# zivy/LSQRRecipes

Measured on AMD Instinct MI355X. Metric: RANSAC hypotheses/sec + final-fit residual, 10M pts, 1/2/4/8 GPU, higher is better.
Workload: dtype f64; 1 GPU; PlaneParametersEstimator + RANSAC, 10000000 points, 50% outliers, delta=0.50 (BASELINE.json configs[1]); points=10000000, streams=4, world_size=1, collectives=none (single GPU), repeats=3

## Files before the change

include/lsqr_hip.h:

```cpp
#ifndef LSQR_HIP_H
#define LSQR_HIP_H

#include <stddef.h>
#include <stdint.h>

#ifdef __cplusplus
extern "C" {
#endif

#if defined(__GNUC__)
#define LSQR_API __attribute__((visibility("default")))
#else
#define LSQR_API
#endif

typedef enum {
  LSQR_OK = 0,
  LSQR_EMPTY = 1,
  LSQR_ERR_INVALID = 2,
  LSQR_ERR_NO_DEVICE = 3,
  LSQR_ERR_HIP = 4,
  LSQR_ERR_STATE = 5
} lsqr_status;

// ... 281 lines not shown
                               uint8_t *consensus_out, lsqr_ransac_info *info);

LSQR_API int lsqr_ransac_exhaustive(lsqr_ctx *ctx, double *params_out, uint8_t *consensus_out,
                                    lsqr_ransac_info *info);
LSQR_API int lsqr_replay_init(size_t n, int k, double p, uint64_t state[6]);
LSQR_API size_t lsqr_replay(size_t n, int k, double p, const uint32_t *subsets,
                            const uint8_t *valid, const uint32_t *votes, size_t H,
                            uint64_t base_index, void *dedup_set, uint64_t state[6]);
LSQR_API void *lsqr_dedup_create(int k);
LSQR_API void lsqr_dedup_destroy(void *set);

LSQR_API int lsqr_set_option(lsqr_ctx *ctx, const char *name, int value);

LSQR_API int lsqr_index_info(const lsqr_ctx *ctx, uint64_t out[4]);

LSQR_API int lsqr_scan_workload(lsqr_ctx *ctx, uint32_t *bound_out, uint64_t out[8]);

LSQR_API int lsqr_scan_work(lsqr_ctx *ctx, uint64_t out[8]);

LSQR_API int lsqr_scan_pairs_counted(lsqr_ctx *ctx, uint64_t out[4]);

LSQR_API int lsqr_lm_persist_info(const lsqr_ctx *ctx, uint64_t out[8], uint64_t *trace, uint32_t trace_cap,
                                  uint32_t *trace_n);

LSQR_API int lsqr_profile_enable(lsqr_ctx *ctx, int on);
LSQR_API int lsqr_profile_get(lsqr_ctx *ctx, int kernel_id, uint64_t *launches, double *total_ms);
LSQR_API int lsqr_profile_reset(lsqr_ctx *ctx);

#ifdef __cplusplus
}
// ... 3 lines not shown
```

lsqrrecipes_amd/_lib.py:

```python
import ctypes as C
import os

import numpy as np

_HERE = os.path.dirname(os.path.abspath(__file__))
LIB_PATH = os.path.join(_HERE, "liblsqr_hip.so")

OK, EMPTY, ERR_INVALID, ERR_NO_DEVICE, ERR_HIP, ERR_STATE = range(6)
PLANE, SPHERE, LINE, DENSE, US_SINGLE, US_POINTER, ABSOR, PIVOT, RAY, LINE2D, PHANTOM = 1, 2, 3, 4, 5, 6, 7, 8, 9, 10, 11
LS_ALGEBRAIC, LS_GEOMETRIC = 0, 1
LS_ANALYTIC, LS_ITERATIVE = 0, 1
KERNEL_IDS = {"sample": 0, "estimate": 1, "scan": 2, "mask": 3, "moments": 4, "solve": 5,
              "index": 6, "absmax": 7}


def assign_dense_chunk(n):
    return 256 if n <= 32 else 128


class LsqrError(RuntimeError):
    def __init__(self, status, msg):
        RuntimeError.__init__(self, "lsqr_hip status %d: %s" % (status, msg))
        self.status = status

# ... 140 lines not shown
    "lsqr_multi_last_error": (C.c_char_p, [C.c_void_p]),
    "lsqr_multi_set_model": (C.c_int, [C.c_void_p, C.POINTER(ModelCfg)]),
    "lsqr_multi_upload": (C.c_int, [C.c_void_p, C.c_void_p, C.c_size_t, C.c_size_t]),
    "lsqr_multi_batch_fit": (C.c_int, [C.c_void_p, C.c_uint64, C.c_uint64, C.c_size_t, C.c_void_p, C.c_void_p,
                                       C.POINTER(RansacInfo)]),
    "lsqr_multi_ransac": (C.c_int, [C.c_void_p, C.c_double, C.c_uint64, C.c_void_p, C.c_void_p,
                                    C.POINTER(RansacInfo)]),
    "lsqr_ransac_exhaustive": (C.c_int, [_ctx, C.c_void_p, C.c_void_p, C.POINTER(RansacInfo)]),
    "lsqr_replay_init": (C.c_int, [C.c_size_t, C.c_int, C.c_double, _u64p]),
    "lsqr_replay": (C.c_size_t, [C.c_size_t, C.c_int, C.c_double, C.c_void_p, C.c_void_p,
                                 C.c_void_p, C.c_size_t, C.c_uint64, C.c_void_p, _u64p]),
    "lsqr_dedup_create": (C.c_void_p, [C.c_int]),
    "lsqr_dedup_destroy": (None, [C.c_void_p]),
    "lsqr_set_option": (C.c_int, [_ctx, C.c_char_p, C.c_int]),
    "lsqr_index_info": (C.c_int, [_ctx, _u64p]),
    "lsqr_scan_workload": (C.c_int, [_ctx, C.c_void_p, _u64p]),
    "lsqr_scan_work": (C.c_int, [_ctx, _u64p]),
    "lsqr_scan_pairs_counted": (C.c_int, [_ctx, _u64p]),
    "lsqr_lm_persist_info": (C.c_int, [_ctx, _u64p, _u64p, C.c_uint32, C.POINTER(C.c_uint32)]),
    "lsqr_profile_enable": (C.c_int, [_ctx, C.c_int]),
    "lsqr_profile_get": (C.c_int, [_ctx, C.c_int, _u64p, _dp]),
    "lsqr_profile_reset": (C.c_int, [_ctx]),
}

_lib = None


def load():
    global _lib
    if _lib is None:
# ... 21 lines not shown
```

lsqrrecipes_amd/context.py:

```python
import ctypes as C

import numpy as np

from . import _lib as L


class Context:
    def __init__(self, device=0):
        self._lib = L.load()
        h = C.c_void_p()
        st = self._lib.lsqr_ctx_create(int(device), C.byref(h))
        if st != L.OK:
            raise L.LsqrError(st, "lsqr_ctx_create(device=%d): %s" % (
                device, self._lib.lsqr_status_string(st).decode()))
        self._h = h
        self.device = device
        self.cfg = None
        self._keep = None

    def close(self):
        if getattr(self, "_h", None):
            self._lib.lsqr_ctx_destroy(self._h)
            self._h = None

# ... 702 lines not shown
        self._chk(self._lib.lsqr_profile_enable(self._h, int(on)))
        self._chk(self._lib.lsqr_profile_reset(self._h))

    def profile_get(self, name):
        n = C.c_uint64(0)
        ms = C.c_double(0)
        self._chk(self._lib.lsqr_profile_get(self._h, L.KERNEL_IDS[name], C.byref(n), C.byref(ms)))
        return n.value, ms.value

    def index_info(self):
        out = (C.c_uint64 * 4)()
        self._chk(self._lib.lsqr_index_info(self._h, out))
        return {"built": bool(out[0]), "observations": int(out[1]), "cells": int(out[2]),
                "cell_points": int(out[3])}

    def scan_workload(self, want_bounds=False):
        H = self._lib.lsqr_num_hypotheses(self._h)
        ub = np.zeros(H, dtype=np.uint32) if want_bounds else None
        out = (C.c_uint64 * 8)()
        self._chk(self._lib.lsqr_scan_workload(self._h, L.ptr(ub), out))
        r = {"pairs": int(out[0]), "level1_evaluations": int(out[1]), "cells": int(out[2]),
             "cell_points": int(out[3]), "bounded": bool(out[4]), "pilots": int(out[5]),
             "second_pass": int(out[6]), "pairs_counted": int(out[7])}
        if want_bounds:
            r["bounds"] = ub
        return r

    def scan_work(self):
        out = (C.c_uint64 * 8)()
        self._chk(self._lib.lsqr_scan_work(self._h, out))
# ... 123 lines not shown
```

lsqrrecipes_amd/csrc/cells.h:

```cpp
#pragma once
#include <hip/hip_runtime.h>
#include <stdint.h>

#include "models.h"

#pragma clang diagnostic ignored "-Winline-asm"

namespace lsqr {

constexpr int kCellPtsMin = 128;
constexpr uint32_t kGroupPad = 4, kCellPad = 16;
constexpr uint32_t kBlockPad = 6;
constexpr uint32_t kQueues = 32;
constexpr uint32_t kQueuePitch = 1088;

struct CellBox {
  float c[3];
  float h[3];
  float pad[2];
};
struct CellSlab {
  float e[3];
  float iee;
  float tmid, tspan;
// ... 1036 lines not shown
      const float a0 = d < D ? (float)(p0[d < D ? d : 0] - off) : 0.0f;
      const float a1 = d < D ? (float)(p1[d < D ? d : 0] - off) : 0.0f;
      xs[p][d].x = (d < D && !(i0 < ns)) ? __builtin_nanf("") : a0;
      xs[p][d].y = (d < D && !(i1 < ns)) ? __builtin_nanf("") : a1;
    }
    v2f q = {0.0f, 0.0f};
    if constexpr (requires { CM::XQ; }) {
      q = xs[p][D - 1] * xs[p][D - 1];
#pragma unroll
      for (int d = D - 2; d >= 0; d--) q = __builtin_elementwise_fma(xs[p][d], xs[p][d], q);
    }
    xs[p][3] = q;
  }
}

template <class CM, int PP, int CPT, int BS, bool LDSB = false>
__global__ __launch_bounds__(BS) __attribute__((amdgpu_waves_per_eu(CPT == 1 ? (PP >= 8 ? 4 : CM::MIN_WAVES) : 1, 8))) void k_scan_cells(const double *__restrict__ sorted, size_t ns,
                                                    const CellBox *__restrict__ boxes,
                                                    uint32_t ncells, const double *__restrict__ sp,
                                                    const float *__restrict__ rows,
                                                    const float *__restrict__ spf, uint32_t H,
                                                    ModelConsts mc, CellConsts cc,
                                                    uint32_t *__restrict__ votes,
                                                    uint32_t *__restrict__ next_tile, uint32_t grab,
                                                    uint32_t hsplit, const uint32_t *__restrict__ h_dev) {
  typedef typename CM::M M;
  constexpr int NB = CM::NB;
  if (h_dev) {
    const uint32_t hd = *h_dev;
    H = hd < H ? hd : H;
  }
  constexpr int SPD = M::SP;
  constexpr int ROW = CM::ROW, NR4 = ROW / 4;
  constexpr int NR2 = CM::ROW2 / 4;
  static_assert(ROW % 4 == 0, "hypothesis rows are fetched as 16-byte loads");
  extern __shared__ uint32_t s_cnt[];
  for (uint32_t h = threadIdx.x; h < H; h += BS) s_cnt[h] = 0;
  __syncthreads();
  const int lane = threadIdx.x & 63;
  float *s_bc = (float *)(s_cnt + ((H + 3) & ~3u)) + (size_t)(threadIdx.x >> 6) * 512;
// ... 27 lines not shown
    const uint32_t hbeg = (un - wt * hsplit) * hseg, hend = hbeg + hseg < H ? hbeg + hseg : H;
    if (hbeg >= H) continue;
    v2f xs[CPT][PP][4];
    CellBox bx[CPT];
    double ctr[CPT][3];
#pragma unroll
    for (int q = 0; q < CPT; q++) {
      const uint32_t cell = wt * CPT + q;
      if (cell < ncells) {
        bx[q] = boxes[cell];
      } else {
        for (int d = 0; d < 3; d++) bx[q].c[d] = 0.0f, bx[q].h[d] = __builtin_nanf("");
      }
#pragma unroll
      for (int d = 0; d < 3; d++) ctr[q][d] = (double)bx[q].c[d];
      cells_load<CM, PP>(sorted, ns, (size_t)cell, lane, ctr[q], xs[q]);
    }
    float4 nxt[NR4];
    {
      const uint32_t hl = hbeg + lane;
      const float4 *r4 = (const float4 *)(rows + (size_t)(hl < H ? hl : 0) * ROW);
#pragma unroll
      for (int k = 0; k < NR4; k++) nxt[k] = r4[k];
    }
    float4 nxt2[NR2 ? NR2 : 1];
    if constexpr (NR2 > 0) {
      const uint32_t hl = hbeg + lane;
      const float4 *r4 = (const float4 *)(spf + (size_t)(hl < H ? hl : 0) * M::SPF + CM::ROW2_OFF);
#pragma unroll
      for (int k = 0; k < NR2; k++) nxt2[k] = r4[k];
    }
// ... 622 lines not shown
    float bc[NB];
    (void)CM::level1(hy, bx, ctr, w.cc, bc);
    base += 64;
    const bool more = base < jhi;
    if (more) hy = hyp_gather<CM>(w.hyps, block_ids(base, s_id + (par ^ 64)));
    cells_filter_squares(bc);
    uint32_t accv = 0;
    cells_survivors<CM, PP, slots_dup(LDSB), Ids::List, EXACT>(
        xs, bc, w.s_bc, surv, lane, w.sorted, w.ns, (size_t)cell, w.sp, w.mc, accv, s_id + par, w.s_amb);
    if (accv) atomicAdd(&w.s_cnt[s_id[par + lane]], accv);
    if (!more) break;
    par ^= 64;
  }
}

template <class CM, int PP, int BS, bool LDSB, PairsForm F>
__global__ __launch_bounds__(BS) __attribute__((amdgpu_waves_per_eu(PP >= 8 ? 4 : CM::MIN_WAVES, 8))) void k_scan_pairs(
    const double *__restrict__ sorted, size_t ns, const CellBox *__restrict__ boxes, uint32_t ncells,
    const double *__restrict__ sp, const float *__restrict__ rows, const float *__restrict__ spf, uint32_t H,
    ModelConsts mc, CellConsts cc, uint32_t *__restrict__ vpart, uint32_t vstride,
    const uint32_t *__restrict__ h_dev, const uint8_t *__restrict__ cnt, uint32_t gstride, const uint32_t *__restrict__ cost,
    const uint32_t *__restrict__ csum, uint32_t nchunks, uint32_t h_off, const float4 *__restrict__ hyps,
    unsigned long long *__restrict__ ambc) {
  static_assert(pairs_form_exists<CM, LDSB, F>());
  constexpr bool PREP = prepared(F), LEAN = lean(F), PACK = packed(F);
  typedef typename CM::M M;
  constexpr int NB = CM::NB;
  constexpr int SPD = M::SP;
  [[maybe_unused]] constexpr int ROW = CM::ROW;
  constexpr int NR2 = CM::ROW2 / 4;
  constexpr int NR4 = [] {
    if constexpr (PREP) return (int)HypWords<CM>::N4;
    else return (int)CM::ROW / 4;
  }();
  if (h_dev) {
    const uint32_t hd = *h_dev > h_off ? *h_dev - h_off : 0u;
    H = hd < H ? hd : H;
  }
  extern __shared__ uint32_t s_cnt[];
// ... 135 lines not shown
    const CellBox bx = boxes[cell];
    double ctr[3];
#pragma unroll
    for (int d = 0; d < 3; d++) ctr[d] = (double)bx.c[d];
    if constexpr (LEAN && PP >= 4) {
#pragma unroll
      for (int d = 0; d < 3; d++) {
        const unsigned long long u = __builtin_bit_cast(unsigned long long, ctr[d]);
        uint32_t l, m;
        asm("s_nop 0\n\tv_readfirstlane_b32 %0, %1\n\ts_nop 1" : "=s"(l) : "v"((uint32_t)u));
        asm("s_nop 0\n\tv_readfirstlane_b32 %0, %1\n\ts_nop 1" : "=s"(m) : "v"((uint32_t)(u >> 32)));
        ctr[d] = __builtin_bit_cast(double, (unsigned long long)m << 32 | l);
      }
    }
    v2f xs[PP][4];
    cells_load<CM, PP>(sorted, ns, (size_t)cell, lane, ctr, xs);
    if constexpr (PACK) {
      pairs_cell_packed<CM, PP, LDSB, recheck(F) ? Exact::Band : Exact::Cell>(w, cell, bx, ctr, xs, jlo, jhi);
      cell++;
      continue;
    }
    if constexpr (LEAN) {
      typename CM::Hyp hy;
      {
        float4 r[NR4], r2[1];
        load_rows((uint32_t)__builtin_ctzll(gm), r, r2);
        hy = hyp_from<CM>(r);
      }
      while (gm && budget) {
        const int g = __builtin_ctzll(gm);
        gm &= gm - 1;
// ... 167 lines not shown
```

lsqrrecipes_amd/csrc/lsqr_hip.hip:

```cpp
#include <hip/hip_runtime.h>

#include <algorithm>
#include <atomic>
#include <chrono>
#include <cmath>
#include <cstdarg>
#include <cstddef>
#include <cstdio>
#include <cstdlib>
#include <cstring>
#include <limits>
#include <set>
#include <thread>
#include <string>
#include <type_traits>
#include <utility>
#include <vector>

#include "../../include/lsqr_hip.h"
#include "devbuf.h"
#include "options.h"
#include "kernels.h"
#include "models_nd.h"
#include "dense.h"
// ... 151 lines not shown

  DevBuf<double> d_sorted;
  DevBuf<uint32_t> d_queues;
  DevBuf<CellBox> d_boxes;
  uint32_t super_merge = 0;
  size_t n_sorted = 0;
  uint32_t n_cells = 0, cell_pts = 0;
  bool index_valid = false;
  bool index_failed = false;
  DevBuf<char> d_idx_scratch;
  int kd_build_levels = 0, index_kd_levels = 0;
  DevBuf<CellAxis> d_axis;
  DevBuf<float> d_cellT;
  bool axis_valid = false;
  DevBuf<CellSlab> d_slab;

  DevBuf<uint32_t> d_ub;
  struct {
    bool valid = false, packed = false, slab = false;
    uint32_t H = 0, h_off = 0, gstride = 0;
    const uint32_t *h_dev = nullptr;
  } last_count;
  DevBuf<uint8_t> d_paircnt;
  DevBuf<uint32_t> d_paircost;
  DevBuf<uint32_t> d_vpart;
  DevBuf<float4> d_hyps;
  DevBuf<unsigned long long> d_pairmask;
  DevBuf<unsigned long long> d_ambcnt;
  bool amb_reset = false;
  bool amb_counted = false;
// ... 438 lines not shown
    if (c->lanes[i]) {
      (void)hipStreamSynchronize(c->lanes[i]->stream);
      for (BatchSlotState &s : c->lanes[i]->slots) s.busy = false;
    }
}

void drop_index(lsqr_ctx *c) {
  c->h16_valid = false;
  c->us16_valid = false;
  c->h16_nomem = c->us16_nomem = false;
  c->n_sorted = 0;
  c->n_cells = 0;
  c->index_valid = false;
  c->index_kd_levels = 0;
  c->axis_valid = false;
  c->last_count.valid = false;
}

template <int D>
int run_bounds(lsqr_ctx *c) {
  if (c->bounds_valid) return LSQR_OK;
  const int nb = grid_for(c->n, 256 * 16, 1024);
  BoundsRow *rows = (BoundsRow *)c->d_partials.get();
  static_assert(sizeof(BoundsRow) == 64, "BoundsRow is 8 words");
  {
    ProfScope ps(c, KID_ABSMAX);
    hipLaunchKernelGGL((k_bounds<D>), dim3(nb), dim3(256), 0, c->stream, c->d_data, c->stride, c->n, rows);
  }
  HIPCHK(c, hipGetLastError());
  hipLaunchKernelGGL(k_bounds_final, dim3(1), dim3(256), 0, c->stream, rows, nb, rows + 1024);
// ... 148 lines not shown
        double xabs;
        memcpy(&xabs, &hb.amax, sizeof xabs);
        hipLaunchKernelGGL(k_cell_slabs, dim3((c->n_cells + 255) / 256), dim3(256), 0, c->stream, c->d_boxes, c->d_axis,
                           c->d_cellT, c->n_sorted, c->n_cells, cell_pts, xabs, (uint32_t)c->opt.slab_gate, c->d_slab);
      }
      IDXCHK(hipGetLastError());
      c->axis_valid = true;
    }
  }
#undef IDXCHK
  c->index_kd_levels = c->kd_build_levels;
  c->index_valid = true;
  return LSQR_OK;
}

struct ScanBatch {
  const double *sp;
  const float *spf;
  size_t H;
  uint32_t *votes;
  const uint32_t *h_dev;
  uint32_t h_off = 0;
};

template <class CM, int PP, int CPT, int BS, bool LDSB = false>
int launch_scan_cells(lsqr_ctx *c, const ScanBatch &b) {
  typedef typename CM::M M;
  const CellConsts cc = cell_consts((const CM *)nullptr, c->mc);
  HIPCHK(c, hipMemsetAsync(b.votes, 0, b.H * sizeof(uint32_t), c->stream));
  if (c->n_cells == 0) return LSQR_OK;
  const size_t wtiles = ((size_t)c->n_cells + CPT - 1) / CPT;
  constexpr int wpb = BS / 64;
  if (!c->d_queues) HIPCHK(c, c->d_queues.alloc(kQueues * kQueuePitch));
  uint32_t *d_next = c->d_queues;
  for (size_t h0 = 0; h0 < b.H; h0 += kScanChunk) {
    uint32_t hc = (uint32_t)std::min<size_t>(kScanChunk, b.H - h0);
    size_t lds = (size_t)((hc + 3) & ~3u) * sizeof(uint32_t) + (LDSB ? (size_t)wpb * 2048 : 0);
    int per_cu = (int)std::min<size_t>(32 / wpb, (160 * 1024) / std::max<size_t>(lds, 1));
    {
      int occ = 0;
      if (hipOccupancyMaxActiveBlocksPerMultiprocessor(&occ, k_scan_cells<CM, PP, CPT, BS, LDSB>, BS, lds) ==
              hipSuccess && occ >= 1)
        per_cu = std::min(per_cu, occ);
      else
        (void)hipGetLastError();
    }
    if (per_cu < 1) per_cu = 1;
    size_t blocks = std::min<size_t>((wtiles + wpb - 1) / wpb, (size_t)256 * per_cu);
    const size_t waves = blocks * wpb, groups = (hc + 63) / 64;
    uint32_t hsplit = 1;
    if (c->opt.hsplit > 0) hsplit = (uint32_t)std::min<size_t>(groups, (size_t)c->opt.hsplit);
    const size_t units = wtiles * hsplit;
    const uint32_t grab = (uint32_t)std::min<size_t>(8, std::max<size_t>(1, units / (32 * waves)));
    ProfScope ps(c, KID_SCAN);
    HIPCHK(c, hipMemsetAsync(d_next, 0, kQueues * kQueuePitch * sizeof(uint32_t), c->stream));
    hipLaunchKernelGGL((k_scan_cells<CM, PP, CPT, BS, LDSB>), dim3((unsigned)blocks), dim3(BS), lds,
                       c->stream, c->d_sorted, c->n_sorted, c->d_boxes, c->n_cells,
                       b.sp + h0 * M::SP,
                       CM::ROW_F32 ? b.spf + h0 * M::SPF : (const float *)(b.sp + h0 * M::SP),
                       b.spf + h0 * M::SPF, hc, c->mc, cc, b.votes + h0, d_next, grab, hsplit, b.h_dev);
    HIPCHK(c, hipGetLastError());
  }
  return LSQR_OK;
}
template <class CM, int PP, int CPT>
int run_scan_cells(lsqr_ctx *c, const ScanBatch &b) {
  if (c->opt.block == 257 || (c->opt.block == 0 && CM::LDS_BROADCAST))
    return launch_scan_cells<CM, PP, CPT, 256, true>(c, b);
  return launch_scan_cells<CM, PP, CPT, 256>(c, b);
}
template <class CM, int PP, int CPT>
int run_scan_cells(lsqr_ctx *c) {
  const ScanBatch b = {c->d_hparams, c->d_hparams_f32, c->H, c->d_votes, nullptr};
  return run_scan_cells<CM, PP, CPT>(c, b);
}

template <class CM, class F>
int with_pp(uint32_t cell_pts, F &&f) {
  if constexpr (requires { CM::MAX_PP; }) {
    if (cell_pts == 1024) return f(std::integral_constant<int, 8>{});
  }
  if (cell_pts == 512) return f(std::integral_constant<int, 4>{});
  return f(std::integral_constant<int, 2>{});
}

template <class CM, int PP>
int run_cells_bounds(lsqr_ctx *c, uint32_t *d_ub, uint32_t *d_nc = nullptr) {
  typedef typename CM::M M;
  const CellConsts cc = cell_consts((const CM *)nullptr, c->mc);
  HIPCHK(c, hipMemsetAsync(d_ub, 0, c->H * sizeof(uint32_t), c->stream));
  if (d_nc) HIPCHK(c, hipMemsetAsync(d_nc, 0, c->H * sizeof(uint32_t), c->stream));
  if (d_nc) HIPCHK(c, hipMemsetAsync(c->d_counter + CNT_PAIRS, 0, sizeof(unsigned long long), c->stream));
  if (c->n_cells == 0) return LSQR_OK;
  uint32_t merge = c->opt.bound_merge ? (uint32_t)c->opt.bound_merge : (uint32_t)CM::BOUND_MERGE;
  if (!c->opt.bound_merge) {
    while (merge > 1 && c->n_cells / merge < 4096) merge /= 2;
    if (c->bsel_known_H && (uint64_t)c->bsel_known.n_rest * 3 > c->bsel_known_H) c->merge_off = true;
    if (c->merge_off) merge = 1;
// ... 65 lines not shown
  }
  const ScanBatch &b = b0;
  const CellConsts cc = cell_consts((const CM *)nullptr, c->mc);
  if (c->n_cells == 0 || b.H == 0) {
    HIPCHK(c, hipMemsetAsync(b.votes, 0, b.H * sizeof(uint32_t), c->stream));
    return LSQR_OK;
  }
  const uint32_t Hc = (uint32_t)b.H, groups = (Hc + 63) / 64;
  const uint32_t gstride = groups <= 1 ? 1u : (groups + 15) / 16 * 16;
  const uint32_t nchunks = (c->n_cells + kChunkCells - 1) / kChunkCells;
  int st;
  if ((st = ensure(c, c->d_paircnt, (size_t)c->n_cells * gstride)) != LSQR_OK) return st;
  if ((st = ensure(c, c->d_paircost, (size_t)c->n_cells + nchunks)) != LSQR_OK) return st;
  uint32_t *d_cost = c->d_paircost, *d_csum = c->d_paircost + c->n_cells;
  const float *rows = CM::ROW_F32 ? b.spf : (const float *)b.sp;
  bool ldsb_default = CM::LDS_BROADCAST;
  if constexpr (requires { CM::LDS_BROADCAST_PAIRS; }) ldsb_default = CM::LDS_BROADCAST_PAIRS;
  const bool ldsb = c->opt.block == 257 || (c->opt.block == 0 && ldsb_default);
  const PairsForm form = pairs_form<CM>(ldsb, c->opt.prepared, c->opt.lean, c->opt.pack, c->opt.recheck);
  if constexpr (cell_prepared<CM>()) {
    if (prepared(form)) {
      const uint32_t slots = (Hc + 63) & ~63u;
      if ((st = ensure(c, c->d_hyps, (size_t)slots * HypWords<CM>::N4)) != LSQR_OK) return st;
      hipLaunchKernelGGL((k_prepare_hyps<CM>), dim3((slots + 255) / 256), dim3(256), 0, c->stream, rows, b.spf, Hc, cc,
                         b.h_dev, b.h_off, c->d_hyps);
      HIPCHK(c, hipGetLastError());
    }
  }
  const float4 *hyps = prepared(form) ? c->d_hyps : nullptr;
  if (packed(form) && (st = ensure(c, c->d_pairmask, (size_t)c->n_cells * gstride)) != LSQR_OK) return st;
  uint8_t *d_cnt = packed(form) ? (uint8_t *)c->d_pairmask.get() : c->d_paircnt.get();
  constexpr int BS = 256, wpb = BS / 64;
  const size_t lds = (size_t)((Hc + 3) & ~3u) * sizeof(uint32_t) + (ldsb ? (size_t)wpb * 2048 : 0) +
// ... 16 lines not shown
                           Hc, cc, per, (uint32_t *)nullptr, (unsigned long long *)nullptr, (uint32_t *)nullptr,
                           d_cnt, gstride, b.h_dev, b.h_off, (uint32_t)(128 * PP), hyps, slabs);
      };
      if (c->opt.lean)
        count(k_cells_bounds<CM, PP, bounds_form(F, true)>);
      else
        count(k_cells_bounds<CM, PP, bounds_form(F, false)>);
      HIPCHK(c, hipGetLastError());
    }
    hipLaunchKernelGGL(k_tile_costs<packed(F)>, dim3(nchunks), dim3(kChunkCells), 0, c->stream, (const uint8_t *)d_cnt,
                       gstride, Hc, b.h_dev, c->n_cells, d_cost, d_csum, b.votes, b.h_off,
                       c->amb_reset ? c->d_ambcnt.get() : (unsigned long long *)nullptr);
    c->amb_reset = false;
    c->amb_counted = cell_prepared<CM>() && M::ND == 3;
    HIPCHK(c, hipGetLastError());
    const auto kern = k_scan_pairs<CM, PP, BS, LDSB, F>;
    int per_cu = (int)std::min<size_t>(32 / wpb, (160 * 1024) / std::max<size_t>(lds, 1)), occ = 0;
    if (hipOccupancyMaxActiveBlocksPerMultiprocessor(&occ, kern, BS, lds) == hipSuccess && occ >= 1)
      per_cu = std::min(per_cu, occ);
    else
      (void)hipGetLastError();
    if (per_cu < 1) per_cu = 1;
    if (c->opt.pairs_waves > 0) per_cu = std::min(per_cu, c->opt.pairs_waves);
    const unsigned blocks = (unsigned)std::min<size_t>(((size_t)c->n_cells + wpb - 1) / wpb, (size_t)256 * per_cu);
    int st2 = ensure(c, c->d_vpart, (size_t)blocks * Hc);
    if (st2 != LSQR_OK) return st2;
    ProfScope ps(c, KID_SCAN);
    hipLaunchKernelGGL(kern, dim3(blocks), dim3(BS), lds, c->stream, c->d_sorted, c->n_sorted, c->d_boxes, c->n_cells,
                       b.sp, rows, b.spf, Hc, c->mc, cc, c->d_vpart, Hc, b.h_dev, (const uint8_t *)d_cnt, gstride,
                       (const uint32_t *)d_cost, (const uint32_t *)d_csum, nchunks, b.h_off, hyps,
                       c->d_ambcnt.get());
    HIPCHK(c, hipGetLastError());
    hipLaunchKernelGGL(k_votes_reduce, dim3((Hc + 63) / 64, 48), dim3(256), 0, c->stream,
                       (const uint32_t *)c->d_vpart, Hc, (uint32_t)blocks, Hc, b.h_dev, b.votes, b.h_off);
    HIPCHK(c, hipGetLastError());
    return LSQR_OK;
  });
}

template <int PP>
int run_rank_bounds(lsqr_ctx *c, const uint32_t **lo_out) {
  typedef PlaneCell<3> CM;
  typedef typename CM::M M;
  const uint32_t H = (uint32_t)c->H;
  int st;
  if (!c->d_ub2) HIPCHK(c, c->d_ub2.alloc(3 * c->H_cap));
  uint32_t *ub2 = c->d_ub2, *lb2 = c->d_ub2 + c->H_cap, *lo = c->d_ub2 + 2 * c->H_cap;
  const CellConsts cc = cell_consts((const CM *)nullptr, c->mc);
  uint32_t *cand = c->d_sel + kPilots;
  double *sp_b = c->d_hparams2 + (size_t)kPilots * M::SP;
  float *spf_b = c->d_hparams2_f32 + (size_t)kPilots * M::SPF;
// ... 634 lines not shown
  uint32_t cell_pts = c->opt.cell ? (uint32_t)c->opt.cell : (uint32_t)CM::DEFAULT_CELL;
  if constexpr (!requires { CM::MAX_PP; }) cell_pts = cell_pts > 512 ? 512 : cell_pts;
  *cell_pts_out = cell_pts;
  int kd_now = c->opt.refine && c->hyp_since_upload >= (uint64_t)c->opt.kd_after ? c->opt.kd_levels : 0;
  if constexpr (std::is_same<CM, PlaneCell<3>>::value) {
    if (CM::USE_BOUND && c->allow_bound && c->opt.bound) kd_now = c->index_kd_levels;
  }
  if (!c->index_valid || c->cell_pts != cell_pts || kd_now > c->index_kd_levels) {
    c->kd_build_levels = kd_now;
    if (build_index<M::ND>(c, cell_pts) != LSQR_OK) {
      (void)hipGetLastError();
      c->index_failed = true;
      return false;
    }
  }
  return true;
}
template <class M>
int scan_plane_key_order(lsqr_ctx *c, uint32_t cell_pts) {
  typedef typename CellOf<M>::type CM;
  const uint32_t H = (uint32_t)c->H;
  uint32_t *perm = c->d_sel + kPilots, *cnt = (uint32_t *)(c->d_counter + CNT_FLAG);
  double *sp_b = c->d_hparams2 + (size_t)kPilots * M::SP;
  float *spf_b = c->d_hparams2_f32 + (size_t)kPilots * M::SPF;
  uint32_t *votes_b = c->d_votes2 + kPilots;
  hipLaunchKernelGGL((k_plane_order<M::SP>), dim3(1), dim3(1024), 0, c->stream, c->d_hparams, H, c->mc.absmax, perm, cnt);
  hipLaunchKernelGGL(k_gather_rows, dim3((H + 3) / 4), dim3(256), 0, c->stream, perm, cnt, H, c->d_hparams, (int)M::SP,
                     c->d_hparams_f32, (int)M::SPF, sp_b, spf_b);
  HIPCHK(c, hipGetLastError());
  const ScanBatch pb = {sp_b, spf_b, (size_t)H, votes_b, nullptr};
// ... 2592 lines not shown
  if (!l) {
    int st = lsqr_ctx_create(c->device, &l);
    if (st != LSQR_OK) return fail(c, st, "cannot create lane %d", li);
    l->is_lane = true;
    if (l->counted) {
      lmp_ctx_count(l->device, -1);
      l->counted = false;
    }
    l->prof = c->prof;
  }
  if (l->lane_epoch != c->data_epoch) {
    if (!c->has_model || !c->d_data) return fail(c, LSQR_ERR_STATE, "no model / records");
    HIPCHK(c, hipStreamSynchronize(l->stream));
    int st = lsqr_set_model(l, &c->cfg);
    l->opt = c->opt;
    if (st == LSQR_OK) st = lsqr_attach(l, c->d_data, c->n, c->stride * sizeof(double));
    if (st != LSQR_OK) return fail(c, st, "lane %d: %s", li, lsqr_last_error(l));
    HIPCHK(c, sync_stream(c));
    l->lane_epoch = c->data_epoch;
  }
  *out = l;
  return LSQR_OK;
}

int lsqr_batch_fit_enqueue(lsqr_ctx *c, uint64_t seed, uint64_t first, size_t H, int slot) {
  if (!c) return LSQR_ERR_INVALID;
  if (!c->is_lane) {
    const int L = lane_count(c);
    if (slot < 0 || slot >= 2 * L) return fail(c, LSQR_ERR_INVALID, "slot %d of %d", slot, 2 * L);
    if (slot % L != 0 || slot / L != slot) {
// ... 695 lines not shown
    MHIP(m, hipStreamSynchronize(c->stream));
  }
  const uint64_t iters = info->iterations, eval = info->evaluated, bidx = info->best_index;
  const uint32_t bv = info->best_votes;
  st = multi_finish(m, seed, rs[RS_BEST_IDX], params_out, consensus_out, info);
  info->iterations = iters;
  info->evaluated = eval;
  info->best_index = bidx;
  info->best_votes = bv;
  if ((st == LSQR_OK || st == LSQR_EMPTY) && info->fit.n_used != bv)
    return mfail(m, LSQR_ERR_HIP, "consensus count of the slices differs from the winner's votes");
  return st;
}

static int apply_option(lsqr_ctx *c, const char *name, int value) {
  bool drops_index = false;
  char why[256];
  const int st = options_set(c->opt, name, value, &drops_index, why, sizeof why);
  if (st == kOptUnknown) return fail(c, LSQR_ERR_INVALID, "unknown option %s", name);
  if (st != LSQR_OK) return fail(c, st, "%s", why);
  if (drops_index) drop_index(c);
  return LSQR_OK;
}
int lsqr_set_option(lsqr_ctx *c, const char *name, int value) {
  if (!c || !name) return LSQR_ERR_INVALID;
  static_assert(lsqr_ctx::kMaxLanes == 4, "the range of batch_lanes' row");
  const bool lanes = !strcmp(name, "batch_lanes");
  if (lanes && value >= 1 && value <= lsqr_ctx::kMaxLanes) {
    bool busy = c->slots[0].busy || c->slots[1].busy;
    for (int i = 1; i < lsqr_ctx::kMaxLanes; i++)
// ... 120 lines not shown
  out[1] = lc.packed ? 1 : 0;
  out[2] = lc.slab ? 1 : 0;
  out[3] = (uint64_t)c->n_cells * lc.H;
  return LSQR_OK;
}

int lsqr_index_info(const lsqr_ctx *c, uint64_t out[4]) {
  if (!c || !out) return LSQR_ERR_INVALID;
  out[0] = c->index_valid ? 1 : 0;
  out[1] = c->n_sorted;
  out[2] = c->n_cells;
  out[3] = c->cell_pts;
  return LSQR_OK;
}

int lsqr_profile_enable(lsqr_ctx *c, int on) {
  if (!c) return LSQR_ERR_INVALID;
  prof_flush(c);
  c->prof = on != 0;
  for (int i = 1; i < lsqr_ctx::kMaxLanes; i++)
    if (c->lanes[i]) lsqr_profile_enable(c->lanes[i], on);
  return LSQR_OK;
}
int lsqr_profile_get(lsqr_ctx *c, int id, uint64_t *launches, double *total_ms) {
  if (!c || id < 0 || id >= 8) return LSQR_ERR_INVALID;
  prof_flush(c);
  uint64_t n = c->launches[id];
  double ms = c->ms[id];
  for (int i = 1; i < lsqr_ctx::kMaxLanes; i++)
    if (c->lanes[i]) {
// ... 22 lines not shown
```

Measured before the change: 7.319 million hypotheses/s.

## Prebuild per-cell fp32 point tiles and load them in scan kernels

When the spatial index is built, a new kernel converts each cell's sorted f64 points into center-relative fp32 tiles laid out for coalesced per-lane vector loads. The cell and pair scan kernels then read these tiles instead of converting from f64 on every visit, which cuts global bytes and conversion work per hypothesis pass. The cost is extra device memory, a one-time build kernel per index, and a fallback to the old path when allocation fails or the configuration spills. A check API and an option to switch it off are added.

```diff
diff --git a/include/lsqr_hip.h b/include/lsqr_hip.h
--- a/include/lsqr_hip.h
+++ b/include/lsqr_hip.h
@@ -319,6 +319,8 @@
 
 LSQR_API int lsqr_index_info(const lsqr_ctx *ctx, uint64_t out[4]);
 
+LSQR_API int lsqr_scan_tiles_check(lsqr_ctx *ctx, uint64_t out[4]);
+
 LSQR_API int lsqr_scan_workload(lsqr_ctx *ctx, uint32_t *bound_out, uint64_t out[8]);
 
 LSQR_API int lsqr_scan_work(lsqr_ctx *ctx, uint64_t out[8]);
diff --git a/lsqrrecipes_amd/_lib.py b/lsqrrecipes_amd/_lib.py
--- a/lsqrrecipes_amd/_lib.py
+++ b/lsqrrecipes_amd/_lib.py
@@ -178,6 +178,7 @@
     "lsqr_dedup_destroy": (None, [C.c_void_p]),
     "lsqr_set_option": (C.c_int, [_ctx, C.c_char_p, C.c_int]),
     "lsqr_index_info": (C.c_int, [_ctx, _u64p]),
+    "lsqr_scan_tiles_check": (C.c_int, [_ctx, _u64p]),
     "lsqr_scan_workload": (C.c_int, [_ctx, C.c_void_p, _u64p]),
     "lsqr_scan_work": (C.c_int, [_ctx, _u64p]),
     "lsqr_scan_pairs_counted": (C.c_int, [_ctx, _u64p]),
diff --git a/lsqrrecipes_amd/context.py b/lsqrrecipes_amd/context.py
--- a/lsqrrecipes_amd/context.py
+++ b/lsqrrecipes_amd/context.py
@@ -740,6 +740,11 @@
         return {"built": bool(out[0]), "observations": int(out[1]), "cells": int(out[2]),
                 "cell_points": int(out[3])}
 
+    def scan_tiles_check(self):
+        out = (C.c_uint64 * 4)()
+        self._chk(self._lib.lsqr_scan_tiles_check(self._h, out))
+        return {"cell_points": int(out[0]), "cells": int(out[1]), "words_differing": int(out[2]), "bytes": int(out[3])}
+
     def scan_workload(self, want_bounds=False):
         H = self._lib.lsqr_num_hypotheses(self._h)
         ub = np.zeros(H, dtype=np.uint32) if want_bounds else None
diff --git a/lsqrrecipes_amd/csrc/cells.h b/lsqrrecipes_amd/csrc/cells.h
--- a/lsqrrecipes_amd/csrc/cells.h
+++ b/lsqrrecipes_amd/csrc/cells.h
@@ -1074,7 +1074,116 @@
   }
 }
 
-template <class CM, int PP, int CPT, int BS, bool LDSB = false>
+template <class CM>
+constexpr int tile_comps() {
+  if constexpr (requires { CM::XQ; }) return CM::M::ND + 1;
+  return CM::M::ND;
+}
+template <class CM>
+constexpr bool tile_paired() {
+  return tile_comps<CM>() % 2 == 0;
+}
+template <class CM>
+constexpr size_t tile_cell_floats(int pp) {
+  return (size_t)128 * pp * tile_comps<CM>();
+}
+template <class CM>
+constexpr int tile_slot(int k) {
+  return k < CM::M::ND ? k : 3;
+}
+typedef float v4f __attribute__((ext_vector_type(4)));
+
+template <class CM, int PP>
+__device__ __forceinline__ void cells_store_tile(float *__restrict__ tiles, const uint32_t cell, const int lane,
+                                                 const v2f (&xs)[PP][4]) {
+  constexpr int NC = tile_comps<CM>();
+  static_assert(NC >= 2 && NC <= 4);
+  float *const base = tiles + (size_t)cell * tile_cell_floats<CM>(PP);
+#pragma unroll
+  for (int p = 0; p < PP; p++) {
+#pragma unroll
+    for (int k = 0; k < NC; k += tile_paired<CM>() ? 2 : 1) {
+      float *const t = base + (p * NC + k) * 128;
+      const v2f a = xs[p][tile_slot<CM>(k)];
+      if constexpr (tile_paired<CM>()) {
+        const v2f b = xs[p][tile_slot<CM>(k + 1)];
+        *(v4f *)(t + 4 * lane) = v4f{a.x, a.y, b.x, b.y};
+      } else {
+        *(v2f *)(t + 2 * lane) = a;
+      }
+    }
+  }
+}
+
+template <class CM, int PP>
+__device__ __forceinline__ void cells_load_tile(const float *__restrict__ tiles, const uint32_t cell, const int lane,
+                                                v2f (&xs)[PP][4]) {
+  constexpr int NC = tile_comps<CM>();
+  static_assert(NC >= 2 && NC <= 4);
+  typedef const __attribute__((address_space(1))) char *gptr;
+  const unsigned long long ra = (unsigned long long)tiles + (unsigned long long)cell * (tile_cell_floats<CM>(PP) * 4);
+  const gptr base = (gptr)((unsigned long long)(uint32_t)__builtin_amdgcn_readfirstlane((int)(uint32_t)(ra >> 32)) << 32 |
+                           (uint32_t)__builtin_amdgcn_readfirstlane((int)(uint32_t)ra));
+  uint32_t off;
+  asm volatile("v_lshlrev_b32 %0, %1, %2" : "=v"(off) : "n"(tile_paired<CM>() ? 4 : 3), "v"(lane));
+#pragma unroll
+  for (int p = 0; p < PP; p++) {
+#pragma unroll
+    for (int k = 0; k < 4; k++) xs[p][k] = v2f{0.0f, 0.0f};
+#pragma unroll
+    for (int k = 0; k < NC; k += tile_paired<CM>() ? 2 : 1) {
+      const gptr t = base + (p * NC + k) * 512 + off;
+      if constexpr (tile_paired<CM>()) {
+        const v4f a = *(const __attribute__((address_space(1))) v4f *)t;
+        xs[p][tile_slot<CM>(k)] = v2f{a.x, a.y};
+        xs[p][tile_slot<CM>(k + 1)] = v2f{a.z, a.w};
+      } else {
+        xs[p][tile_slot<CM>(k)] = *(const __attribute__((address_space(1))) v2f *)t;
+      }
+    }
+  }
+}
+
+template <class CM, int PP>
+__global__ __launch_bounds__(256) void k_build_tiles(const double *__restrict__ sorted, size_t ns,
+                                                     const CellBox *__restrict__ boxes, uint32_t ncells,
+                                                     float *__restrict__ tiles) {
+  const int lane = threadIdx.x & 63;
+  const uint32_t cell = blockIdx.x * 4 + (threadIdx.x >> 6);
+  if (cell >= ncells) return;
+  const CellBox bx = boxes[cell];
+  double ctr[3];
+#pragma unroll
+  for (int d = 0; d < 3; d++) ctr[d] = (double)bx.c[d];
+  v2f xs[PP][4];
+  cells_load<CM, PP>(sorted, ns, (size_t)cell, lane, ctr, xs);
+  cells_store_tile<CM, PP>(tiles, cell, lane, xs);
+}
+template <class CM, int PP>
+__global__ __launch_bounds__(256) void k_check_tiles(const double *__restrict__ sorted, size_t ns,
+                                                     const CellBox *__restrict__ boxes, uint32_t ncells,
+                                                     const float *__restrict__ tiles, unsigned long long *bad) {
+  const int lane = threadIdx.x & 63;
+  const uint32_t cell = blockIdx.x * 4 + (threadIdx.x >> 6);
+  if (cell >= ncells) return;
+  const CellBox bx = boxes[cell];
+  double ctr[3];
+#pragma unroll
+  for (int d = 0; d < 3; d++) ctr[d] = (double)bx.c[d];
+  v2f xa[PP][4], xb[PP][4];
+  cells_load<CM, PP>(sorted, ns, (size_t)cell, lane, ctr, xa);
+  cells_load_tile<CM, PP>(tiles, cell, lane, xb);
+  uint32_t n = 0;
+#pragma unroll
+  for (int p = 0; p < PP; p++)
+#pragma unroll
+    for (int k = 0; k < 4; k++)
+      n += (__builtin_bit_cast(uint32_t, xa[p][k].x) != __builtin_bit_cast(uint32_t, xb[p][k].x)) +
+           (__builtin_bit_cast(uint32_t, xa[p][k].y) != __builtin_bit_cast(uint32_t, xb[p][k].y));
+  if (n) atomicAdd(bad, (unsigned long long)n);
+}
+
+template <class CM, int PP, int CPT, int BS, bool LDSB = false, class... TILES>
 __global__ __launch_bounds__(BS) __attribute__((amdgpu_waves_per_eu(CPT == 1 ? (PP >= 8 ? 4 : CM::MIN_WAVES) : 1, 8))) void k_scan_cells(const double *__restrict__ sorted, size_t ns,
                                                     const CellBox *__restrict__ boxes,
                                                     uint32_t ncells, const double *__restrict__ sp,
@@ -1083,7 +1192,9 @@
                                                     ModelConsts mc, CellConsts cc,
                                                     uint32_t *__restrict__ votes,
                                                     uint32_t *__restrict__ next_tile, uint32_t grab,
-                                                    uint32_t hsplit, const uint32_t *__restrict__ h_dev) {
+                                                    uint32_t hsplit, const uint32_t *__restrict__ h_dev,
+                                                    TILES... tiles) {
+  static_assert(sizeof...(TILES) <= 1);
   typedef typename CM::M M;
   constexpr int NB = CM::NB;
   if (h_dev) {
@@ -1141,7 +1252,10 @@
       }
 #pragma unroll
       for (int d = 0; d < 3; d++) ctr[q][d] = (double)bx[q].c[d];
-      cells_load<CM, PP>(sorted, ns, (size_t)cell, lane, ctr[q], xs[q]);
+      if constexpr (sizeof...(TILES) != 0)
+        cells_load_tile<CM, PP>(tiles..., cell, lane, xs[q]);
+      else
+        cells_load<CM, PP>(sorted, ns, (size_t)cell, lane, ctr[q], xs[q]);
     }
     float4 nxt[NR4];
     {
@@ -1794,15 +1908,16 @@
   }
 }
 
-template <class CM, int PP, int BS, bool LDSB, PairsForm F>
+template <class CM, int PP, int BS, bool LDSB, PairsForm F, class... TILES>
 __global__ __launch_bounds__(BS) __attribute__((amdgpu_waves_per_eu(PP >= 8 ? 4 : CM::MIN_WAVES, 8))) void k_scan_pairs(
     const double *__restrict__ sorted, size_t ns, const CellBox *__restrict__ boxes, uint32_t ncells,
     const double *__restrict__ sp, const float *__restrict__ rows, const float *__restrict__ spf, uint32_t H,
     ModelConsts mc, CellConsts cc, uint32_t *__restrict__ vpart, uint32_t vstride,
     const uint32_t *__restrict__ h_dev, const uint8_t *__restrict__ cnt, uint32_t gstride, const uint32_t *__restrict__ cost,
     const uint32_t *__restrict__ csum, uint32_t nchunks, uint32_t h_off, const float4 *__restrict__ hyps,
-    unsigned long long *__restrict__ ambc) {
+    unsigned long long *__restrict__ ambc, TILES... tiles) {
   static_assert(pairs_form_exists<CM, LDSB, F>());
+  static_assert(sizeof...(TILES) <= 1);
   constexpr bool PREP = prepared(F), LEAN = lean(F), PACK = packed(F);
   typedef typename CM::M M;
   constexpr int NB = CM::NB;
@@ -1968,7 +2083,10 @@
       }
     }
     v2f xs[PP][4];
-    cells_load<CM, PP>(sorted, ns, (size_t)cell, lane, ctr, xs);
+    if constexpr (sizeof...(TILES) != 0)
+      cells_load_tile<CM, PP>(tiles..., cell, lane, xs);
+    else
+      cells_load<CM, PP>(sorted, ns, (size_t)cell, lane, ctr, xs);
     if constexpr (PACK) {
       pairs_cell_packed<CM, PP, LDSB, recheck(F) ? Exact::Band : Exact::Cell>(w, cell, bx, ctr, xs, jlo, jhi);
       cell++;
diff --git a/lsqrrecipes_amd/csrc/lsqr_hip.hip b/lsqrrecipes_amd/csrc/lsqr_hip.hip
--- a/lsqrrecipes_amd/csrc/lsqr_hip.hip
+++ b/lsqrrecipes_amd/csrc/lsqr_hip.hip
@@ -189,6 +189,10 @@
   DevBuf<float> d_cellT;
   bool axis_valid = false;
   DevBuf<CellSlab> d_slab;
+  DevBuf<float> d_tiles;
+  uint32_t tiles_pts = 0;
+  bool tiles_nomem = false;
+  bool use_tiles = true;
 
   DevBuf<uint32_t> d_ub;
   struct {
@@ -657,6 +661,8 @@
   c->index_valid = false;
   c->index_kd_levels = 0;
   c->axis_valid = false;
+  c->tiles_pts = 0;
+  c->tiles_nomem = false;
   c->last_count.valid = false;
 }
 
@@ -835,6 +841,17 @@
   return LSQR_OK;
 }
 
+inline const float *scan_tiles(const lsqr_ctx *c, uint32_t cell_pts) {
+  return c->use_tiles && c->tiles_pts == cell_pts && c->cell_pts == cell_pts ? c->d_tiles.get() : nullptr;
+}
+template <class CM, int PP>
+constexpr bool kTileSpills = std::is_same<CM, PlaneCell<3>>::value && PP == 4;
+template <class CM, int PP, int CPT, bool LDSB>
+constexpr bool kTileScanCells = CPT == 1 && LDSB == (CM::LDS_BROADCAST != 0) && !kTileSpills<CM, PP>;
+template <class CM, int PP, bool LDSB, bool LDSB_DEFAULT, PairsForm F>
+constexpr bool kTileScanPairs = (cell_prepared<CM>() ? packed(F) : F == PairsForm::General) && LDSB == LDSB_DEFAULT &&
+                                !(kTileSpills<CM, PP> && F == PairsForm::Packed);
+
 struct ScanBatch {
   const double *sp;
   const float *spf;
@@ -854,14 +871,13 @@
   constexpr int wpb = BS / 64;
   if (!c->d_queues) HIPCHK(c, c->d_queues.alloc(kQueues * kQueuePitch));
   uint32_t *d_next = c->d_queues;
-  for (size_t h0 = 0; h0 < b.H; h0 += kScanChunk) {
+  auto chunk = [&](auto kern, const size_t h0, auto... tiles) -> int {
     uint32_t hc = (uint32_t)std::min<size_t>(kScanChunk, b.H - h0);
     size_t lds = (size_t)((hc + 3) & ~3u) * sizeof(uint32_t) + (LDSB ? (size_t)wpb * 2048 : 0);
     int per_cu = (int)std::min<size_t>(32 / wpb, (160 * 1024) / std::max<size_t>(lds, 1));
     {
       int occ = 0;
-      if (hipOccupancyMaxActiveBlocksPerMultiprocessor(&occ, k_scan_cells<CM, PP, CPT, BS, LDSB>, BS, lds) ==
-              hipSuccess && occ >= 1)
+      if (hipOccupancyMaxActiveBlocksPerMultiprocessor(&occ, kern, BS, lds) == hipSuccess && occ >= 1)
         per_cu = std::min(per_cu, occ);
       else
         (void)hipGetLastError();
@@ -875,12 +891,24 @@
     const uint32_t grab = (uint32_t)std::min<size_t>(8, std::max<size_t>(1, units / (32 * waves)));
     ProfScope ps(c, KID_SCAN);
     HIPCHK(c, hipMemsetAsync(d_next, 0, kQueues * kQueuePitch * sizeof(uint32_t), c->stream));
-    hipLaunchKernelGGL((k_scan_cells<CM, PP, CPT, BS, LDSB>), dim3((unsigned)blocks), dim3(BS), lds,
-                       c->stream, c->d_sorted, c->n_sorted, c->d_boxes, c->n_cells,
+    hipLaunchKernelGGL(kern, dim3((unsigned)blocks), dim3(BS), lds,
+                       c->stream, c->d_sorted.get(), c->n_sorted, c->d_boxes.get(), c->n_cells,
                        b.sp + h0 * M::SP,
                        CM::ROW_F32 ? b.spf + h0 * M::SPF : (const float *)(b.sp + h0 * M::SP),
-                       b.spf + h0 * M::SPF, hc, c->mc, cc, b.votes + h0, d_next, grab, hsplit, b.h_dev);
+                       b.spf + h0 * M::SPF, hc, c->mc, cc, b.votes + h0, d_next, grab, hsplit, b.h_dev, tiles...);
     HIPCHK(c, hipGetLastError());
+    return LSQR_OK;
+  };
+  [[maybe_unused]] const float *tiles = scan_tiles(c, (uint32_t)(128 * PP));
+  for (size_t h0 = 0; h0 < b.H; h0 += kScanChunk) {
+    int st;
+    if constexpr (kTileScanCells<CM, PP, CPT, LDSB>) {
+      st = tiles ? chunk(k_scan_cells<CM, PP, CPT, BS, LDSB, const float *>, h0, tiles)
+                 : chunk(k_scan_cells<CM, PP, CPT, BS, LDSB>, h0);
+    } else {
+      st = chunk(k_scan_cells<CM, PP, CPT, BS, LDSB>, h0);
+    }
+    if (st != LSQR_OK) return st;
   }
   return LSQR_OK;
 }
@@ -903,6 +931,25 @@
   }
   if (cell_pts == 512) return f(std::integral_constant<int, 4>{});
   return f(std::integral_constant<int, 2>{});
+}
+
+template <class CM>
+int build_tiles(lsqr_ctx *c) {
+  if (!c->use_tiles || !c->index_valid || c->n_cells == 0 || c->tiles_pts == c->cell_pts || c->tiles_nomem) return LSQR_OK;
+  const size_t need = (size_t)c->n_cells * tile_cell_floats<CM>((int)(c->cell_pts / 128));
+  if (need > c->d_tiles.cap() && c->d_tiles.alloc(need) != hipSuccess) {
+    (void)hipGetLastError();
+    c->tiles_nomem = true;
+    return LSQR_OK;
+  }
+  const int st = with_pp<CM>(c->cell_pts, [&](auto pp) -> int {
+    hipLaunchKernelGGL((k_build_tiles<CM, decltype(pp)::value>), dim3((c->n_cells + 3) / 4), dim3(256), 0, c->stream,
+                       c->d_sorted.get(), c->n_sorted, c->d_boxes.get(), c->n_cells, c->d_tiles.get());
+    HIPCHK(c, hipGetLastError());
+    return LSQR_OK;
+  });
+  if (st == LSQR_OK) c->tiles_pts = c->cell_pts;
+  return st;
 }
 
 template <class CM, int PP>
@@ -998,9 +1045,11 @@
   if ((st = ensure(c, c->d_paircost, (size_t)c->n_cells + nchunks)) != LSQR_OK) return st;
   uint32_t *d_cost = c->d_paircost, *d_csum = c->d_paircost + c->n_cells;
   const float *rows = CM::ROW_F32 ? b.spf : (const float *)b.sp;
-  bool ldsb_default = CM::LDS_BROADCAST;
-  if constexpr (requires { CM::LDS_BROADCAST_PAIRS; }) ldsb_default = CM::LDS_BROADCAST_PAIRS;
-  const bool ldsb = c->opt.block == 257 || (c->opt.block == 0 && ldsb_default);
+  constexpr bool kLdsbDefault = [] {
+    if constexpr (requires { CM::LDS_BROADCAST_PAIRS; }) return CM::LDS_BROADCAST_PAIRS != 0;
+    else return CM::LDS_BROADCAST != 0;
+  }();
+  const bool ldsb = c->opt.block == 257 || (c->opt.block == 0 && kLdsbDefault);
   const PairsForm form = pairs_form<CM>(ldsb, c->opt.prepared, c->opt.lean, c->opt.pack, c->opt.recheck);
   if constexpr (cell_prepared<CM>()) {
     if (prepared(form)) {
@@ -1047,27 +1096,33 @@
     c->amb_reset = false;
     c->amb_counted = cell_prepared<CM>() && M::ND == 3;
     HIPCHK(c, hipGetLastError());
-    const auto kern = k_scan_pairs<CM, PP, BS, LDSB, F>;
-    int per_cu = (int)std::min<size_t>(32 / wpb, (160 * 1024) / std::max<size_t>(lds, 1)), occ = 0;
-    if (hipOccupancyMaxActiveBlocksPerMultiprocessor(&occ, kern, BS, lds) == hipSuccess && occ >= 1)
-      per_cu = std::min(per_cu, occ);
-    else
-      (void)hipGetLastError();
-    if (per_cu < 1) per_cu = 1;
-    if (c->opt.pairs_waves > 0) per_cu = std::min(per_cu, c->opt.pairs_waves);
-    const unsigned blocks = (unsigned)std::min<size_t>(((size_t)c->n_cells + wpb - 1) / wpb, (size_t)256 * per_cu);
-    int st2 = ensure(c, c->d_vpart, (size_t)blocks * Hc);
-    if (st2 != LSQR_OK) return st2;
-    ProfScope ps(c, KID_SCAN);
-    hipLaunchKernelGGL(kern, dim3(blocks), dim3(BS), lds, c->stream, c->d_sorted, c->n_sorted, c->d_boxes, c->n_cells,
-                       b.sp, rows, b.spf, Hc, c->mc, cc, c->d_vpart, Hc, b.h_dev, (const uint8_t *)d_cnt, gstride,
-                       (const uint32_t *)d_cost, (const uint32_t *)d_csum, nchunks, b.h_off, hyps,
-                       c->d_ambcnt.get());
-    HIPCHK(c, hipGetLastError());
-    hipLaunchKernelGGL(k_votes_reduce, dim3((Hc + 63) / 64, 48), dim3(256), 0, c->stream,
-                       (const uint32_t *)c->d_vpart, Hc, (uint32_t)blocks, Hc, b.h_dev, b.votes, b.h_off);
-    HIPCHK(c, hipGetLastError());
-    return LSQR_OK;
+    auto scan = [&](auto kern, auto... tiles) -> int {
+      int per_cu = (int)std::min<size_t>(32 / wpb, (160 * 1024) / std::max<size_t>(lds, 1)), occ = 0;
+      if (hipOccupancyMaxActiveBlocksPerMultiprocessor(&occ, kern, BS, lds) == hipSuccess && occ >= 1)
+        per_cu = std::min(per_cu, occ);
+      else
+        (void)hipGetLastError();
+      if (per_cu < 1) per_cu = 1;
+      if (c->opt.pairs_waves > 0) per_cu = std::min(per_cu, c->opt.pairs_waves);
+      const unsigned blocks = (unsigned)std::min<size_t>(((size_t)c->n_cells + wpb - 1) / wpb, (size_t)256 * per_cu);
+      int st2 = ensure(c, c->d_vpart, (size_t)blocks * Hc);
+      if (st2 != LSQR_OK) return st2;
+      ProfScope ps(c, KID_SCAN);
+      hipLaunchKernelGGL(kern, dim3(blocks), dim3(BS), lds, c->stream, c->d_sorted.get(), c->n_sorted, c->d_boxes.get(),
+                         c->n_cells, b.sp, rows, b.spf, Hc, c->mc, cc, c->d_vpart.get(), Hc, b.h_dev, (const uint8_t *)d_cnt,
+                         gstride, (const uint32_t *)d_cost, (const uint32_t *)d_csum, nchunks, b.h_off, hyps,
+                         c->d_ambcnt.get(), tiles...);
+      HIPCHK(c, hipGetLastError());
+      hipLaunchKernelGGL(k_votes_reduce, dim3((Hc + 63) / 64, 48), dim3(256), 0, c->stream,
+                         (const uint32_t *)c->d_vpart, Hc, (uint32_t)blocks, Hc, b.h_dev, b.votes, b.h_off);
+      HIPCHK(c, hipGetLastError());
+      return LSQR_OK;
+    };
+    if constexpr (kTileScanPairs<CM, PP, LDSB, kLdsbDefault, F>) {
+      if (const float *tiles = scan_tiles(c, (uint32_t)(128 * PP)))
+        return scan(k_scan_pairs<CM, PP, BS, LDSB, F, const float *>, tiles);
+    }
+    return scan(k_scan_pairs<CM, PP, BS, LDSB, F>);
   });
 }
 
@@ -1732,6 +1787,7 @@
       return false;
     }
   }
+  if (build_tiles<CM>(c) != LSQR_OK) (void)hipGetLastError();
   return true;
 }
 template <class M>
@@ -4354,6 +4410,7 @@
     HIPCHK(c, hipStreamSynchronize(l->stream));
     int st = lsqr_set_model(l, &c->cfg);
     l->opt = c->opt;
+    l->use_tiles = c->use_tiles;
     if (st == LSQR_OK) st = lsqr_attach(l, c->d_data, c->n, c->stride * sizeof(double));
     if (st != LSQR_OK) return fail(c, st, "lane %d: %s", li, lsqr_last_error(l));
     HIPCHK(c, sync_stream(c));
@@ -5079,6 +5136,12 @@
 }
 
 static int apply_option(lsqr_ctx *c, const char *name, int value) {
+  if (!strcmp(name, "scan_tiles")) {
+    if (value < 0 || value > 1)
+      return fail(c, LSQR_ERR_INVALID, "scan_tiles does not accept %d (0 or 1: the scans open a cell from the index's fp32 tiles)", value);
+    c->use_tiles = value != 0;
+    return LSQR_OK;
+  }
   bool drops_index = false;
   char why[256];
   const int st = options_set(c->opt, name, value, &drops_index, why, sizeof why);
@@ -5229,6 +5292,39 @@
   return LSQR_OK;
 }
 
+int lsqr_scan_tiles_check(lsqr_ctx *c, uint64_t out[4]) {
+  int st = need_ready(c, true);
+  if (st != LSQR_OK) return st;
+  if (!out) return fail(c, LSQR_ERR_INVALID, "null argument");
+  out[0] = c->index_valid ? c->tiles_pts : 0;
+  out[1] = c->n_cells;
+  out[2] = out[3] = 0;
+  if (!out[0] || c->n_cells == 0) return LSQR_OK;
+  unsigned long long *d_bad = c->d_counter + CNT_SUM;
+  HIPCHK(c, hipMemsetAsync(d_bad, 0, sizeof(unsigned long long), c->stream));
+  st = dispatch(c->cfg, [&](auto tag) -> int {
+    typedef typename decltype(tag)::type M;
+    if constexpr (requires { typename CellOf<M>::type; }) {
+      typedef typename CellOf<M>::type CM;
+      out[3] = (uint64_t)c->n_cells * tile_cell_floats<CM>((int)(c->tiles_pts / 128)) * sizeof(float);
+      return with_pp<CM>(c->tiles_pts, [&](auto pp) -> int {
+        hipLaunchKernelGGL((k_check_tiles<CM, decltype(pp)::value>), dim3((c->n_cells + 3) / 4), dim3(256), 0, c->stream,
+                           c->d_sorted.get(), c->n_sorted, c->d_boxes.get(), c->n_cells, c->d_tiles.get(), d_bad);
+        HIPCHK(c, hipGetLastError());
+        return LSQR_OK;
+      });
+    } else {
+      return fail(c, LSQR_ERR_INVALID, "model has no two-level scan");
+    }
+  });
+  if (st != LSQR_OK) return st;
+  unsigned long long *pin = c->h_pin->scratch_u64;
+  HIPCHK(c, hipMemcpyAsync(pin, d_bad, sizeof(unsigned long long), hipMemcpyDeviceToHost, c->stream));
+  HIPCHK(c, sync_stream(c));
+  out[2] = pin[0];
+  return LSQR_OK;
+}
+
 int lsqr_profile_enable(lsqr_ctx *c, int on) {
   if (!c) return LSQR_ERR_INVALID;
   prof_flush(c);
```

Result: faster. 7.477 million hypotheses/s, median of 6 (+2.2%).
